# melspectrum007/audio-visual-speech-enhancement

Hardware: NVIDIA B200
Metric: audio-sec/sec (higher is better)
Workload: dtype f32

## Files before the change

audio-visual-speech-enhancement_b200/csrc/avse_common.h:

```cpp
#pragma once

#if defined(__CUDACC__)
#define AVSE_HD __host__ __device__ __forceinline__
#define AVSE_HD_COLD __host__ __device__ __noinline__
#else
#define AVSE_HD inline
#define AVSE_HD_COLD inline
#endif

namespace avse {

constexpr int NFFT = 640;
constexpr int HOP = 160;
constexpr int NBINS = NFFT / 2 + 1;
constexpr int NMEL = 80;
constexpr int SPSS = 20;
constexpr int HALF = NFFT / 2;

constexpr int N1 = 16;
constexpr int N2 = 40;

constexpr int FPG = 2;
constexpr int ROW_F = 84;
constexpr int FRAME_ZERO_F = N1 * ROW_F;
constexpr int FRAME_FLUSH_F = N1 * ROW_F + 16;
constexpr int FRAME_F = FRAME_FLUSH_F + 96;
constexpr int SCAN_BINS = 336;
constexpr int MEL_STAGE_F = 3 * NMEL * FPG;
constexpr int WARP_SMEM_F = FPG * FRAME_F;
static_assert(MEL_STAGE_F <= FRAME_F, "mel staging must fit in one frame buffer");

constexpr int MEL_WMAX = 24;
constexpr int MEL_WROW = 28;
constexpr int MEL_ROUNDS = NMEL / 16;
constexpr int POST_CHUNK = 21;

constexpr float AMIN = 1e-5f;
constexpr float TOP_DB = 80.0f;

#if !defined(AVSE_SPLIT_BLOCKS_FIRST)
#define AVSE_SPLIT_BLOCKS_FIRST 0
#endif
struct WarpSplit {
    long long base;
    int q, r;
    long long extras;
};
inline WarpSplit make_warp_split(long long total, long long blocks, int warps) {
    WarpSplit s;
    const long long nw = blocks * warps;
    s.base = total / nw;
    s.extras = total % nw;
    s.q = (int)(s.extras / blocks);
    s.r = (int)(s.extras % blocks);
    return s;
}
AVSE_HD void warp_split_range(const WarpSplit& s, int block, int warp, int warps, long long& first, long long& count) {
#if AVSE_SPLIT_BLOCKS_FIRST
    const int eb = s.q + (block < s.r ? 1 : 0);
    first = ((long long)block * warps + warp) * s.base + (long long)block * s.q + (block < s.r ? block : s.r) + (warp < eb ? warp : eb);
    count = s.base + (warp < eb ? 1 : 0);
#else
    const long long gw = (long long)block * warps + warp;
    first = gw * s.base + (gw < s.extras ? gw : s.extras);
    count = s.base + (gw < s.extras ? 1 : 0);
#endif
}

#if defined(__CUDACC__)
template <int N4, int THREADS>
struct TableRegs {
    static constexpr int K = (N4 + THREADS - 1) / THREADS;
    float4 v[K];
};
template <int N4, int THREADS>
__device__ __forceinline__ void table_fetch(const void* g, int tid, TableRegs<N4, THREADS>& r) {
#pragma unroll
    for (int k = 0; k < TableRegs<N4, THREADS>::K; ++k) {
        const int i = tid + k * THREADS;
        r.v[k] = i < N4 ? __ldg(reinterpret_cast<const float4*>(g) + i) : make_float4(0.0f, 0.0f, 0.0f, 0.0f);
    }
}
template <int N4, int THREADS>
__device__ __forceinline__ void table_put(float* s, int tid, const TableRegs<N4, THREADS>& r) {
#pragma unroll
    for (int k = 0; k < TableRegs<N4, THREADS>::K; ++k) {
        const int i = tid + k * THREADS;
        if (i < N4) reinterpret_cast<float4*>(s)[i] = r.v[k];
    }
}
template <int N4, int THREADS>
__device__ __forceinline__ void table_put_scaled(float* s, int tid, const TableRegs<N4, THREADS>& r, float scale) {
#pragma unroll
    for (int k = 0; k < TableRegs<N4, THREADS>::K; ++k) {
        const int i = tid + k * THREADS;
        if (i < N4) reinterpret_cast<float4*>(s)[i] = make_float4(r.v[k].x * scale, r.v[k].y * scale, r.v[k].z * scale, r.v[k].w * scale);
    }
}
#endif

}
```

audio-visual-speech-enhancement_b200/csrc/avse_kernels.cu:

```cuda
#include <cuda_runtime.h>
#include <cooperative_groups.h>
#include <cstdio>
#include <cstring>
#include <cstdlib>
#include <string>
#include <vector>
#include <new>

#include "../../include/avse_b200.h"
#include "avse_common.h"
#include "avse_tables.h"
#include "avse_ctx.h"
#include "avse_fwd_stages.cuh"
#include "avse_fwd4_stages.cuh"

using namespace avse;

static thread_local std::string g_err;
int avse_fail(int code, const std::string& msg) { g_err = msg; return code; }
int avse_cuda_fail(cudaError_t e, const char* where) {
    g_err = std::string(where) + ": " + cudaGetErrorString(e);
    return (int)e;
}

// ... 92 lines not shown
    return 0;
}

extern "C" int avse_get_geometry(const avse_ctx* ctx, int* out6) {
    if (ctx == nullptr || out6 == nullptr) return avse_fail(AVSE_E_ARG, "avse_get_geometry: NULL argument");
    out6[0] = ctx->n_fft; out6[1] = ctx->hop; out6[2] = ctx->n_bins; out6[3] = ctx->n_mels; out6[4] = ctx->spss;
    out6[5] = ctx->generic ? 1 : 0;
    return 0;
}

extern "C" int avse_create_ex(int sample_rate, int n_fft, int hop, int n_mels, int spss, double fmin, double fmax, int device,
                              avse_ctx** out) {
    const char* fg = getenv("AVSE_FORCE_GENERIC");
    if (n_fft == NFFT && hop == HOP && n_mels == NMEL && spss == SPSS && !(fg != nullptr && fg[0] == '1')) {
        const int rc = avse_create(sample_rate, fmin, fmax, device, out);
        if (rc != AVSE_E_CONFIG) return rc;
    }
    if (out == nullptr) return avse_fail(AVSE_E_ARG, "avse_create_ex: out is NULL");
    *out = nullptr;
    avse_ctx* c = new (std::nothrow) avse_ctx();
    if (c == nullptr) return avse_fail(AVSE_E_ARG, "avse_create_ex: out of host memory");
    if (!build_generic(c->gen, sample_rate, n_fft, hop, n_mels, spss, fmin, fmax)) {
        std::string e = c->gen.error;
        delete c;
        return avse_fail(AVSE_E_CONFIG, "avse_create_ex: " + e);
    }
    int ndev = 0;
    cudaError_t e = cudaGetDeviceCount(&ndev);
    if (e != cudaSuccess || ndev == 0) { delete c; return avse_fail(AVSE_E_NOCUDA, "avse_create_ex: no CUDA device (this library has no CPU path)"); }
    if (device < 0 || device >= ndev) { delete c; return avse_fail(AVSE_E_ARG, "avse_create_ex: bad device index"); }
    c->device = device;
    c->generic = true;
    c->n_fft = n_fft; c->hop = hop; c->n_bins = c->gen.geo.bins; c->n_mels = n_mels; c->spss = spss;
    int prev = 0;
    cudaGetDevice(&prev);
    CUDA_TRY(cudaSetDevice(device));
    cudaDeviceGetAttribute(&c->num_sms, cudaDevAttrMultiProcessorCount, device);
    const GenericHost& h = c->gen;
    struct Sec { const void* src; size_t bytes; size_t off; };
    std::vector<Sec> secs = {
        {h.window.data(), h.window.size() * 4, 0},         {h.tw.data(), h.tw.size() * 8, 0},
        {h.window_inv.data(), h.window_inv.size() * 4, 0}, {h.tw_inv.data(), h.tw_inv.size() * 8, 0},
        {h.band_lo.data(), h.band_lo.size() * 4, 0},       {h.band_cnt.data(), h.band_cnt.size() * 4, 0},
        {h.band_off.data(), h.band_off.size() * 4, 0},     {h.band_w.data(), h.band_w.size() * 4, 0},
        {h.pinv.data(), h.pinv.size() * 4, 0},
    };
    size_t total = 0;
    for (auto& sc : secs) { sc.off = total; total += (sc.bytes + 255) / 256 * 256; }
    std::vector<char> stage(total, 0);
    for (auto& sc : secs) memcpy(stage.data() + sc.off, sc.src, sc.bytes);
    e = cudaMalloc(&c->gbase, total);
    if (e != cudaSuccess) { delete c; cudaSetDevice(prev); return avse_cuda_fail(e, "cudaMalloc(generic tables)"); }
    e = cudaMemcpy(c->gbase, stage.data(), total, cudaMemcpyHostToDevice);
    if (e != cudaSuccess) { cudaFree(c->gbase); delete c; cudaSetDevice(prev); return avse_cuda_fail(e, "cudaMemcpy(generic tables)"); }
    char* b = (char*)c->gbase;
    c->gd.window = (const float*)(b + secs[0].off);
    c->gd.tw = (const double*)(b + secs[1].off);
    c->gd.window_inv = (const float*)(b + secs[2].off);
    c->gd.tw_inv = (const double*)(b + secs[3].off);
    c->gd.band_lo = (const int*)(b + secs[4].off);
    c->gd.band_cnt = (const int*)(b + secs[5].off);
    c->gd.band_off = (const int*)(b + secs[6].off);
    c->gd.band_w = (const float*)(b + secs[7].off);
    c->gd.pinv = (const float*)(b + secs[8].off);
    cudaSetDevice(prev);
    *out = c;
    return 0;
}

template <typename S> struct Sample4;
template <> struct Sample4<float> {
    typedef float4 vec;
    static __device__ __forceinline__ void load(const float* p, int i, float (&v)[4]) {
        const float4 t = __ldg(reinterpret_cast<const float4*>(p) + i); v[0] = t.x; v[1] = t.y; v[2] = t.z; v[3] = t.w;
    }
};
template <> struct Sample4<short> {
    typedef short4 vec;
    static __device__ __forceinline__ void load(const short* p, int i, float (&v)[4]) {
        const short4 t = __ldg(reinterpret_cast<const short4*>(p) + i); v[0] = t.x; v[1] = t.y; v[2] = t.z; v[3] = t.w;
    }
};

template <typename S, bool CLUSTER>
__global__ void __launch_bounds__(256) avse_snr_factor_kernel(const S* __restrict__ speech, const S* __restrict__ noise,
                                                              long long stride, const int* __restrict__ lengths,
                                                              const int* __restrict__ noise_period, int L,
                                                              const float* __restrict__ snr_db, float* __restrict__ factor_out,
                                                              float* __restrict__ equalizer_out, int* __restrict__ max_key,
                                                              int* __restrict__ min_key) {
    namespace cg = cooperative_groups;
    cg::cluster_group cluster = cg::this_cluster();
    const int P = CLUSTER ? (int)cluster.num_blocks() : 1;
    const int part = CLUSTER ? (int)cluster.block_rank() : 0;
    const int u = blockIdx.x / P;
    int n = lengths ? lengths[u] : L;
    n = n < 0 ? 0 : (n > L ? L : n);
    int Pn = noise_period ? noise_period[u] : n;
    Pn = (Pn <= 0 || Pn > n) ? n : Pn;
    const int q = Pn > 0 ? n / Pn : 0, rem = Pn > 0 ? n - q * Pn : 0;
    const S* s = speech + (size_t)u * stride;
    const S* z = noise + (size_t)u * stride;
    double a0 = 0.0, a1 = 0.0, b0 = 0.0, b1 = 0.0;
    constexpr size_t AL = sizeof(typename Sample4<S>::vec) - 1;
    const int n4 = ((((size_t)s | (size_t)z) & AL) == 0) ? (n >> 2) : 0;
    const int per4 = (n4 + P - 1) / P;
    const int lo4 = part * per4, hi4 = lo4 + per4 < n4 ? lo4 + per4 : n4;
    if (Pn == n) {
        for (int i = lo4 + threadIdx.x; i < hi4; i += blockDim.x) {
            float sv[4], zv[4];
            Sample4<S>::load(s, i, sv);
            Sample4<S>::load(z, i, zv);
            a0 += (double)sv[0] + (double)sv[1] + (double)sv[2] + (double)sv[3];
            a1 += (double)sv[0] * sv[0] + (double)sv[1] * sv[1] + (double)sv[2] * sv[2] + (double)sv[3] * sv[3];
            b0 += (double)zv[0] + (double)zv[1] + (double)zv[2] + (double)zv[3];
            b1 += (double)zv[0] * zv[0] + (double)zv[1] * zv[1] + (double)zv[2] * zv[2] + (double)zv[3] * zv[3];
        }
        if (part == P - 1)
            for (int i = 4 * n4 + threadIdx.x; i < n; i += blockDim.x) {
                const double sv = (double)s[i], zv = (double)z[i];
                a0 += sv; a1 += sv * sv; b0 += zv; b1 += zv * zv;
            }
    } else {
        for (int i = lo4 + threadIdx.x; i < hi4; i += blockDim.x) {
            float sv[4];
            Sample4<S>::load(s, i, sv);
            a0 += (double)sv[0] + (double)sv[1] + (double)sv[2] + (double)sv[3];
            a1 += (double)sv[0] * sv[0] + (double)sv[1] * sv[1] + (double)sv[2] * sv[2] + (double)sv[3] * sv[3];
        }
        if (part == P - 1)
            for (int i = 4 * n4 + threadIdx.x; i < n; i += blockDim.x) { const double sv = (double)s[i]; a0 += sv; a1 += sv * sv; }
        const int perp = (Pn + P - 1) / P;
        const int lop = part * perp, hip = lop + perp < Pn ? lop + perp : Pn;
        for (int i = lop + threadIdx.x; i < hip; i += blockDim.x) {
            const double zv = (double)z[i], w = (double)(q + (i < rem ? 1 : 0));
            b0 += w * zv; b1 += w * zv * zv;
        }
    }
    __shared__ double red[4][8];
    __shared__ double partial[4];
#pragma unroll
    for (int o = 16; o > 0; o >>= 1) {
        a0 += __shfl_xor_sync(0xffffffffu, a0, o);
        a1 += __shfl_xor_sync(0xffffffffu, a1, o);
        b0 += __shfl_xor_sync(0xffffffffu, b0, o);
        b1 += __shfl_xor_sync(0xffffffffu, b1, o);
    }
    const int w = threadIdx.x >> 5, l = threadIdx.x & 31;
    if (l == 0) { red[0][w] = a0; red[1][w] = a1; red[2][w] = b0; red[3][w] = b1; }
    __syncthreads();
    if (threadIdx.x < 4) {
        double t = 0.0;
        for (int i = 0; i < 8; ++i) t += red[threadIdx.x][i];
        partial[threadIdx.x] = t;
    }
    if (CLUSTER) cluster.sync();
    else __syncthreads();
    if (part == 0 && threadIdx.x == 0) {
        double t[4] = {0.0, 0.0, 0.0, 0.0};
        for (int r = 0; r < P; ++r) {
            const double* qq = CLUSTER ? cluster.map_shared_rank(partial, r) : partial;
            t[0] += qq[0]; t[1] += qq[1]; t[2] += qq[2]; t[3] += qq[3];
        }
        float g = 0.0f, f = 0.0f;
        if (n > 0) {
            const double inv = 1.0 / (double)n;
            const double ms = t[0] * inv, mn = t[2] * inv;
            const double vs = t[1] * inv - ms * ms, vn = t[3] * inv - mn * mn;
            const double db = snr_db ? (double)snr_db[u] : 0.0;
            const double eq = sqrt(vs / vn);
            g = (float)eq;
            f = (float)(eq * pow(10.0, -db / 20.0));
        }
        factor_out[u] = f;
        if (equalizer_out) equalizer_out[u] = g;
        if (max_key) { max_key[3 * u] = (int)0x80000000; max_key[3 * u + 1] = (int)0x80000000; max_key[3 * u + 2] = (int)0x80000000; }
        if (min_key) { min_key[3 * u] = 0x7fffffff; min_key[3 * u + 1] = 0x7fffffff; min_key[3 * u + 2] = 0x7fffffff; }
    }
    if (CLUSTER) cluster.sync();
}

template <typename S>
static cudaError_t launch_snr_factor(int B, int P, cudaStream_t st, const S* speech, const S* noise, long long stride, const int* lengths,
                                     const int* noise_period, int L, const float* snr_db, float* factor_out, float* equalizer_out,
                                     int* max_key, int* min_key) {
    if (P == 1) {
        avse_snr_factor_kernel<S, false><<<B, 256, 0, st>>>(speech, noise, stride, lengths, noise_period, L, snr_db, factor_out,
                                                            equalizer_out, max_key, min_key);
        return cudaGetLastError();
    }
    cudaLaunchConfig_t cfg = {};
    cfg.gridDim = dim3((unsigned)(B * P));
    cfg.blockDim = dim3(256);
    cfg.dynamicSmemBytes = 0;
    cfg.stream = st;
    cudaLaunchAttribute attr[1];
    attr[0].id = cudaLaunchAttributeClusterDimension;
    attr[0].val.clusterDim.x = (unsigned)P;
    attr[0].val.clusterDim.y = 1;
    attr[0].val.clusterDim.z = 1;
    cfg.attrs = attr;
    cfg.numAttrs = 1;
    return cudaLaunchKernelEx(&cfg, avse_snr_factor_kernel<S, true>, speech, noise, stride, lengths, noise_period, L, snr_db, factor_out,
                              equalizer_out, max_key, min_key);
}

extern "C" int avse_snr_factor(avse_ctx* ctx, const void* speech, const void* noise, int sample_format, long long stride,
                               const int* lengths, const int* noise_period, int B, int L, const float* snr_db, float* factor_out,
                               float* equalizer_out, int* max_key, int* min_key, void* stream) {
    if (!ctx || !speech || !noise || !factor_out) return avse_fail(AVSE_E_ARG, "avse_snr_factor: NULL argument");
    if (B <= 0 || L <= 0 || stride < L) return avse_fail(AVSE_E_ARG, "avse_snr_factor: bad sizes");
    int P = 1;
    while (P < 8 && (long long)B * P < 4LL * ctx->num_sms && L / (2 * P) >= 65536) P *= 2;
    cudaError_t e;
    if (sample_format == AVSE_SAMPLE_F32)
        e = launch_snr_factor<float>(B, P, (cudaStream_t)stream, (const float*)speech, (const float*)noise, stride, lengths, noise_period, L,
                                     snr_db, factor_out, equalizer_out, max_key, min_key);
    else if (sample_format == AVSE_SAMPLE_I16)
        e = launch_snr_factor<short>(B, P, (cudaStream_t)stream, (const short*)speech, (const short*)noise, stride, lengths, noise_period, L,
                                     snr_db, factor_out, equalizer_out, max_key, min_key);
    else return avse_fail(AVSE_E_ARG, "avse_snr_factor: bad sample_format");
    if (e != cudaSuccess) return avse_cuda_fail(e, "avse_snr_factor launch");
    CUDA_TRY(cudaGetLastError());
    return 0;
}

#ifndef AVSE_FWD_WARPS
#define AVSE_FWD_WARPS 8
#endif
#ifndef AVSE_FWD_CTAS
#define AVSE_FWD_CTAS 2
#endif
constexpr int FWD_WARPS = AVSE_FWD_WARPS;
constexpr int FWD_CTAS = AVSE_FWD_CTAS;
constexpr int FWD_THREADS = FWD_WARPS * 32;
constexpr int FWD_SM_WIN = FWD_WARPS * WARP_SMEM_F;
constexpr int FWD_SM_TW = FWD_SM_WIN + 2 * NFFT;
constexpr int FWD_SM_MODE = FWD_SM_TW + N1 * N2 * 2;
constexpr int FWD_SM_SCANW = FWD_SM_MODE;
constexpr int FWD_SM_SCANMASK = FWD_SM_SCANW + SCAN_BINS * 4;
constexpr int FWD_SM_SCANLOC = FWD_SM_SCANMASK + 16;
constexpr int FWD_SM_MELW = FWD_SM_MODE;
constexpr int FWD_SM_MELLO = FWD_SM_MELW + NMEL * MEL_WROW;
constexpr int FWD_SM_ROUNDW = FWD_SM_MELLO + NMEL;
constexpr int FWD_SMEM_F_SCAN = FWD_SM_SCANLOC + NMEL * 4;
constexpr int FWD_SMEM_F_GEN = FWD_SM_ROUNDW + 16;
constexpr int FWD_SMEM_F = FWD_SMEM_F_GEN > FWD_SMEM_F_SCAN ? FWD_SMEM_F_GEN : FWD_SMEM_F_SCAN;
constexpr int FWD_SMEM_BYTES = FWD_SMEM_F * 4;
static_assert((FWD_SM_MODE % 4) == 0 && (FWD_SM_TW % 2) == 0 && (FWD_SM_SCANLOC % 4) == 0, "table alignment");
static_assert(FWD_CTAS * (FWD_SMEM_BYTES + 1024) <= 233472, "the resident CTAs must fit in shared memory");

struct MixGain { float gain, resid; };
static __device__ __forceinline__ MixGain mix_gain(const avse_forward_args& A, int u) {
    const float f = A.factor ? A.factor[u] : 1.0f;
    MixGain m;
    if (A.equalizer) { m.gain = A.equalizer[u]; m.resid = m.gain != 0.0f ? __fdividef(f, m.gain) : 0.0f; }
    else { m.gain = f; m.resid = 1.0f; }
    return m;
}

struct FwdParams {
    avse_forward_args a;
    FwdTables tb;
    int T;
    int G;
    int total_tiles;
    int per_warp;
    WarpSplit split;
};

template <bool SCAN>
__global__ void __launch_bounds__(FWD_THREADS, FWD_CTAS) avse_forward_kernel(const __grid_constant__ FwdParams P) {
    extern __shared__ __align__(16) float smem[];
    const int warp = threadIdx.x >> 5, lane = threadIdx.x & 31;
    if (SCAN) {
        for (int i = threadIdx.x; i < SCAN_BINS * 4; i += FWD_THREADS) smem[FWD_SM_SCANW + i] = P.tb.scan_w[i];
        if (threadIdx.x < 16) reinterpret_cast<int*>(smem + FWD_SM_SCANMASK)[threadIdx.x] = P.tb.scan_mask[threadIdx.x];
        for (int i = threadIdx.x; i < NMEL * 4; i += FWD_THREADS) reinterpret_cast<int*>(smem + FWD_SM_SCANLOC)[i] = P.tb.scan_loc[i];
    } else {
        for (int i = threadIdx.x; i < NMEL * MEL_WROW; i += FWD_THREADS) smem[FWD_SM_MELW + i] = P.tb.mel_w[i];
        for (int i = threadIdx.x; i < NMEL; i += FWD_THREADS) reinterpret_cast<int*>(smem + FWD_SM_MELLO)[i] = P.tb.mel_lo[i];
        if (threadIdx.x < MEL_ROUNDS) reinterpret_cast<int*>(smem + FWD_SM_ROUNDW)[threadIdx.x] = P.tb.mel_roundw[threadIdx.x];
    }
    for (int i = threadIdx.x; i < 2 * NFFT; i += FWD_THREADS) smem[FWD_SM_WIN + i] = P.tb.window2[i];
    for (int i = threadIdx.x; i < N1 * N2 * 2; i += FWD_THREADS) smem[FWD_SM_TW + i] = P.tb.tw1t[i];
    float* frames = smem + warp * WARP_SMEM_F;
    for (int i = lane; i < WARP_SMEM_F; i += 32) frames[i] = 0.0f;
    __syncthreads();

    const float* s_melw = smem + FWD_SM_MELW;
    const int* s_mello = reinterpret_cast<const int*>(smem + FWD_SM_MELLO);
    const int* s_roundw = reinterpret_cast<const int*>(smem + FWD_SM_ROUNDW);
    const float* s_win = smem + FWD_SM_WIN;
    const vec2* s_tw = reinterpret_cast<const vec2*>(smem + FWD_SM_TW);

    const avse_forward_args& A = P.a;
    const bool have_noise = A.noise != nullptr;
    const int gw = blockIdx.x * FWD_WARPS + warp;
    int tile = gw * P.per_warp;
    int n_tiles = P.total_tiles - tile;
    n_tiles = n_tiles < P.per_warp ? n_tiles : P.per_warp;
    if (n_tiles <= 0) return;
// ... 98 lines not shown
#pragma unroll
                for (int q = 0; q < 3; ++q) stage_db_scan(lane, q, factor, have_noise, s_loc, frames, out, g * FPG, P.T, mx);
            } else {
#pragma unroll
                for (int q = 0; q < 3; ++q) stage_db(lane, q, factor, have_noise, frames, out, g * FPG, P.T, mx);
            }
        }
        __syncwarp();

        if (++g == P.G) {
            flush_max(u);
            g = 0;
            ++u;
            fresh = true;
        }
    }
    if (!fresh) flush_max(u);
}


#ifndef AVSE_P1_UNIFIED
#define AVSE_P1_UNIFIED 0
#endif
#ifndef AVSE_F4_PREFETCH
#define AVSE_F4_PREFETCH 2
#endif
#ifndef AVSE_F4_WARPS
#define AVSE_F4_WARPS 8
#endif
constexpr int F4_WARPS = AVSE_F4_WARPS;
constexpr int F4_THREADS = F4_WARPS * 32;
constexpr int F4_SM_WIN = F4_WARPS * WARP4_SMEM_F;
constexpr int F4_SM_TW = F4_SM_WIN + NFFT;
constexpr int F4_SM_SCANW = F4_SM_TW + N1 * N2 * 2;
constexpr int F4_SM_LOC = F4_SM_SCANW + SCAN4_BINS * 2;
constexpr int F4_SM_MIN = F4_SM_LOC + NMEL * 4;
#ifndef AVSE_F4_PTR_SLOT
#define AVSE_F4_PTR_SLOT 1
#endif
constexpr int F4_UTT_F = AVSE_F4_PTR_SLOT ? 12 : 2;
constexpr int F4_SM_UTT = F4_SM_MIN + F4_WARPS * 96;
constexpr int F4_SMEM_F = F4_SM_UTT + F4_WARPS * 2 * F4_UTT_F;
constexpr int F4_SMEM_BYTES = F4_SMEM_F * 4;
static_assert((F4_SM_TW % 2) == 0 && (F4_SM_SCANW % 2) == 0 && (F4_SM_LOC % 4) == 0 && (F4_SM_UTT % 4) == 0, "table alignment");
static_assert(F4_SMEM_BYTES + 1024 <= 232448, "F4 shared memory must fit in one SM");

#ifndef AVSE_F4_BATCHED_PROLOGUE
#define AVSE_F4_BATCHED_PROLOGUE 1
#endif
__device__ __noinline__ void f4_fill_tables(float* smem, float* frames, const float* window, const float* tw1t, const float* scan4_w,
                                            const int* scan4_loc) {
    static_assert((F4_SM_WIN % 4) == 0 && (F4_SM_TW % 4) == 0 && (F4_SM_SCANW % 4) == 0 && (F4_SM_LOC % 4) == 0 && (WARP4_SMEM_F % 4) == 0, "16-byte table copies");
    const int tid = threadIdx.x, lane = threadIdx.x & 31;
    TableRegs<NFFT / 4, F4_THREADS> r_win;
    TableRegs<N1 * N2 * 2 / 4, F4_THREADS> r_tw;
    TableRegs<SCAN4_BINS * 2 / 4, F4_THREADS> r_sw;
    TableRegs<NMEL, F4_THREADS> r_loc;
    table_fetch(window, tid, r_win);
    table_fetch(tw1t, tid, r_tw);
    table_fetch(scan4_w, tid, r_sw);
    table_fetch(scan4_loc, tid, r_loc);
    for (int i = lane; i < WARP4_SMEM_F / 4; i += 32) reinterpret_cast<float4*>(frames)[i] = make_float4(0.0f, 0.0f, 0.0f, 0.0f);
    table_put(smem + F4_SM_WIN, tid, r_win);
    table_put(smem + F4_SM_TW, tid, r_tw);
    table_put(smem + F4_SM_SCANW, tid, r_sw);
    table_put(smem + F4_SM_LOC, tid, r_loc);
}

template <typename S, bool TILED, bool PAD>
__global__ void __launch_bounds__(F4_THREADS, 1) avse_forward4_kernel(const __grid_constant__ FwdParams P) {
    extern __shared__ __align__(16) float smem[];
    const int warp = threadIdx.x >> 5, lane = threadIdx.x & 31;
    float* frames = smem + warp * WARP4_SMEM_F;
#if AVSE_F4_BATCHED_PROLOGUE
    f4_fill_tables(smem, frames, P.tb.window, P.tb.tw1t, P.tb.scan4_w, P.tb.scan4_loc);
#else
    for (int i = threadIdx.x; i < NFFT; i += F4_THREADS) smem[F4_SM_WIN + i] = P.tb.window[i];
    for (int i = threadIdx.x; i < N1 * N2 * 2; i += F4_THREADS) smem[F4_SM_TW + i] = P.tb.tw1t[i];
    for (int i = threadIdx.x; i < SCAN4_BINS * 2; i += F4_THREADS) smem[F4_SM_SCANW + i] = P.tb.scan4_w[i];
    for (int i = threadIdx.x; i < NMEL * 4; i += F4_THREADS) reinterpret_cast<int*>(smem + F4_SM_LOC)[i] = P.tb.scan4_loc[i];
    for (int i = lane; i < WARP4_SMEM_F; i += 32) frames[i] = 0.0f;
#endif
    __syncthreads();

    const float* s_win = smem + F4_SM_WIN;
    const vec2* s_tw = reinterpret_cast<const vec2*>(smem + F4_SM_TW);
    const vec2* s_scanw = reinterpret_cast<const vec2*>(smem + F4_SM_SCANW);
    const ivec4* s_loc = reinterpret_cast<const ivec4*>(smem + F4_SM_LOC);

    Lane4Const lc;
    lane4_const_init(lane, s_win, s_tw, lc);
    const unsigned mask_lo = P.tb.scan4_mask[2 * (lane & 7)], mask_hi = P.tb.scan4_mask[2 * (lane & 7) + 1];

    const avse_forward_args& A = P.a;
    long long first, count;
    warp_split_range(P.split, (int)blockIdx.x, warp, F4_WARPS, first, count);
    int tile = (int)first;
    const int n_tiles = (int)count;
    if (n_tiles <= 0) return;
    int u = tile / P.G;
    int g = tile - u * P.G;

    float mx[3] = {neg_inf(), neg_inf(), neg_inf()};
    float* mn = smem + F4_SM_MIN + warp * 96;
    mn[lane] = -neg_inf(); mn[32 + lane] = -neg_inf(); mn[64 + lane] = -neg_inf();
    float factor = 0.0f;
    int vs = 0, vn = 0;
    float* utt_sm = smem + F4_SM_UTT + warp * (2 * F4_UTT_F);
    const S* in_speech = reinterpret_cast<const S*>(A.speech);
    const S* in_noise = reinterpret_cast<const S*>(A.noise);
    constexpr int LINE = 128 / (int)sizeof(S);

    auto flush_max = [&](int uu) {
#pragma unroll
        for (int s = 0; s < 3; ++s) {
            float v = mx[s], w = mn[32 * s + lane];
#pragma unroll
            for (int o = 16; o > 0; o >>= 1) {
                v = fmaxf(v, __shfl_xor_sync(0xffffffffu, v, o));
                w = fminf(w, __shfl_xor_sync(0xffffffffu, w, o));
            }
            if (lane == 0) {
                atomicMax(A.max_key + 3 * uu + s, float_to_key(v));
                if (A.min_key) atomicMin(A.min_key + 3 * uu + s, float_to_key(w));
            }
            mx[s] = neg_inf();
            mn[32 * s + lane] = -neg_inf();
        }
    };

    auto prefetch_ahead = [&](int it, int u, int g) {
#if AVSE_F4_PREFETCH > 0
        if (it + AVSE_F4_PREFETCH < n_tiles) {
            int g2 = g + AVSE_F4_PREFETCH, u2 = u;
            if (g2 >= P.G) { g2 -= P.G; ++u2; }
            const int lo = g2 == 0 ? 0 : g2 * (F4 * HOP) + HOP;
            const int hi = g2 * (F4 * HOP) + (NFFT + HOP);
            const int i0 = (lo & ~(LINE - 1)) + LINE * lane;
            if (i0 < hi && i0 < A.L && i0 < A.in_stride && lane < 22) {
                const size_t o = (size_t)u2 * A.in_stride + i0;
                asm volatile("prefetch.global.L2 [%0];" ::"l"(in_speech + o));
                asm volatile("prefetch.global.L2 [%0];" ::"l"(in_noise + o));
            }
        }
#endif
    };
    auto load_utt = [&](int uu, int& ovs, int& ovn, float& of) {
        ovs = A.len_speech ? A.len_speech[uu] : A.L;
        ovn = A.len_noise ? A.len_noise[uu] : ovs;
        ovs = ovs < 0 ? 0 : (ovs < A.L ? ovs : A.L);
        ovn = ovn < 0 ? 0 : (ovn < A.L ? ovn : A.L);
        const MixGain mg = mix_gain(A, uu);
        of = mg.resid;
        utt_sm[F4_UTT_F * (uu & 1)] = mg.gain;
#if AVSE_F4_PTR_SLOT
        {
            float** ps = reinterpret_cast<float**>(utt_sm + F4_UTT_F * (uu & 1) + 2);
            ps[0] = A.out_speech ? A.out_speech + (size_t)uu * A.out_stride : nullptr;
            ps[1] = A.out_noise ? A.out_noise + (size_t)uu * A.out_stride : nullptr;
            ps[2] = A.out_mixed ? A.out_mixed + (size_t)uu * A.out_stride : nullptr;
            ps[3] = A.mixed_pcm ? A.mixed_pcm + (size_t)uu * A.pcm_stride : nullptr;
        }
#endif
        if (TILED) {
            int period = A.noise_period[uu];
            if (period <= 0 || period >= ovn) period = 0;
// ... 93 lines not shown
            out.dst[1] = A.out_noise ? A.out_noise + (size_t)u * A.out_stride : nullptr;
            out.dst[2] = A.out_mixed ? A.out_mixed + (size_t)u * A.out_stride : nullptr;
#endif
            out.layout = A.layout;
            out.n_slices = A.n_slices;
            out.ld_t = A.ld_t;
#pragma unroll 1
#if AVSE_DB_SPLIT_LAST && AVSE_DB_BRANCHFREE_EXTRA
            for (int q = 0; q < 2; ++q) stage4_db(lane, q, tl.factor, s_loc, frames, out, g * F4, P.T, mx, mn);
            stage4_db_last(lane, tl.factor, s_loc, frames, out, g * F4, P.T, mx, mn);
#else
            for (int q = 0; q < 3; ++q) stage4_db(lane, q, tl.factor, s_loc, frames, out, g * F4, P.T, mx, mn);
#endif
        }
        __syncwarp();

        if (last_of_utt || !have_next) flush_max(u);
        u = u2; g = g2; vs = vs2; vn = vn2;
        tl = tnx;
        interior = interior2;
        reflect = reflect2;
    }
}

__global__ void avse_reset_max_kernel(int* __restrict__ max_key, int* __restrict__ min_key, int n, int min_value);

extern "C" int avse_forward(avse_ctx* ctx, const avse_forward_args* args, void* stream) {
    if (!ctx || !args) return avse_fail(AVSE_E_ARG, "avse_forward: NULL argument");
    if (ctx->generic) return avse_generic_forward(ctx, args, stream);
    const avse_forward_args& a = *args;
    if (!a.speech || !a.max_key) return avse_fail(AVSE_E_ARG, "avse_forward: speech and max_key are required");
    if (a.B <= 0 || a.L <= HALF) return avse_fail(AVSE_E_ARG, "avse_forward: need B > 0 and L > 320 (reflect padding)");
    if (!a.len_speech && a.in_stride < a.L) return avse_fail(AVSE_E_ARG, "avse_forward: in_stride < L needs len_speech");
    if (a.layout != AVSE_LAYOUT_SLICES && a.layout != AVSE_LAYOUT_SPEC) return avse_fail(AVSE_E_ARG, "avse_forward: bad layout");
    FwdParams P;
    P.a = a;
    P.tb = ctx->fwd;
    P.T = 1 + a.L / HOP;
    P.G = (P.T + FPG - 1) / FPG;
    if (a.layout == AVSE_LAYOUT_SLICES) {
        if (a.n_slices < 0 || (long long)a.n_slices * AVSE_SPSS > P.T) return avse_fail(AVSE_E_ARG, "avse_forward: n_slices exceeds int(T/20) (dp:50)");
        if (a.out_stride < (long long)a.n_slices * NMEL * AVSE_SPSS) return avse_fail(AVSE_E_ARG, "avse_forward: out_stride too small");
    } else {
        if (a.ld_t < P.T) return avse_fail(AVSE_E_ARG, "avse_forward: ld_t < T");
        if (a.out_stride < (long long)NMEL * a.ld_t) return avse_fail(AVSE_E_ARG, "avse_forward: out_stride too small");
    }
    if (a.mixed_pcm && a.pcm_stride < a.L) return avse_fail(AVSE_E_ARG, "avse_forward: pcm_stride < L");
    float* outs[3] = {a.out_speech, a.out_noise, a.out_mixed};
    for (int s = 0; s < 3; ++s)
        if (outs[s] && (((size_t)outs[s] & 15) || (a.out_stride & 3))) return avse_fail(AVSE_E_ARG, "avse_forward: outputs must be 16-byte aligned with out_stride % 4 == 0");
    const long long total = (long long)a.B * P.G;
    if (total > 0x7fffffffLL) return avse_fail(AVSE_E_ARG, "avse_forward: B * groups exceeds 2^31; split the batch");

    static thread_local int configured_dev = -1;
    int dev = 0;
    CUDA_TRY(cudaGetDevice(&dev));
    if (dev != ctx->device) return avse_fail(AVSE_E_ARG, "avse_forward: current device differs from the context's device");
    if (a.sample_format != AVSE_SAMPLE_F32 && a.sample_format != AVSE_SAMPLE_I16) return avse_fail(AVSE_E_ARG, "avse_forward: bad sample_format");
    const bool i16 = a.sample_format == AVSE_SAMPLE_I16;
    const bool use_f4 = ctx->f4_tables && a.noise != nullptr && a.stft_speech == nullptr && (!ctx->force_f2 || i16);
    if (i16 && !use_f4) return avse_fail(AVSE_E_ARG, "avse_forward: int16 samples are supported for pair batches (noise != NULL, no stft_speech) with the standard 2-tap filterbank; convert to float32 first");
    if (use_f4) {
        static thread_local int configured4_dev = -1;
        if (configured4_dev != dev) {
            CUDA_TRY(cudaFuncSetAttribute(avse_forward4_kernel<float, false, false>, cudaFuncAttributeMaxDynamicSharedMemorySize, F4_SMEM_BYTES));
            CUDA_TRY(cudaFuncSetAttribute(avse_forward4_kernel<short, false, false>, cudaFuncAttributeMaxDynamicSharedMemorySize, F4_SMEM_BYTES));
            CUDA_TRY(cudaFuncSetAttribute(avse_forward4_kernel<float, false, true>, cudaFuncAttributeMaxDynamicSharedMemorySize, F4_SMEM_BYTES));
            CUDA_TRY(cudaFuncSetAttribute(avse_forward4_kernel<short, false, true>, cudaFuncAttributeMaxDynamicSharedMemorySize, F4_SMEM_BYTES));
            CUDA_TRY(cudaFuncSetAttribute(avse_forward4_kernel<float, true, false>, cudaFuncAttributeMaxDynamicSharedMemorySize, F4_SMEM_BYTES));
            CUDA_TRY(cudaFuncSetAttribute(avse_forward4_kernel<short, true, false>, cudaFuncAttributeMaxDynamicSharedMemorySize, F4_SMEM_BYTES));
            configured4_dev = dev;
        }
        P.G = (P.T + F4 - 1) / F4;
        const long long total4 = (long long)a.B * P.G;
        long long blocks4 = ctx->num_sms;
        const long long need4 = (total4 + F4_WARPS - 1) / F4_WARPS;
        if (blocks4 > need4) blocks4 = need4;
        const long long nwarps4 = blocks4 * F4_WARPS;
        P.total_tiles = (int)total4;
        P.per_warp = (int)((total4 + nwarps4 - 1) / nwarps4);
        P.split = make_warp_split(total4, blocks4, F4_WARPS);
        const bool tiled = a.noise_period != nullptr;
        const bool pad = !tiled && (a.len_speech != nullptr || a.len_noise != nullptr);
        const cudaStream_t st4 = (cudaStream_t)stream;
        if (i16 && tiled) avse_forward4_kernel<short, true, false><<<(unsigned)blocks4, F4_THREADS, F4_SMEM_BYTES, st4>>>(P);
        else if (tiled) avse_forward4_kernel<float, true, false><<<(unsigned)blocks4, F4_THREADS, F4_SMEM_BYTES, st4>>>(P);
        else if (i16 && pad) avse_forward4_kernel<short, false, true><<<(unsigned)blocks4, F4_THREADS, F4_SMEM_BYTES, st4>>>(P);
        else if (pad) avse_forward4_kernel<float, false, true><<<(unsigned)blocks4, F4_THREADS, F4_SMEM_BYTES, st4>>>(P);
        else if (i16) avse_forward4_kernel<short, false, false><<<(unsigned)blocks4, F4_THREADS, F4_SMEM_BYTES, st4>>>(P);
        else avse_forward4_kernel<float, false, false><<<(unsigned)blocks4, F4_THREADS, F4_SMEM_BYTES, st4>>>(P);
        CUDA_TRY(cudaGetLastError());
        return 0;
    }
    if (configured_dev != dev) {
        CUDA_TRY(cudaFuncSetAttribute(avse_forward_kernel<true>, cudaFuncAttributeMaxDynamicSharedMemorySize, FWD_SMEM_BYTES));
        CUDA_TRY(cudaFuncSetAttribute(avse_forward_kernel<false>, cudaFuncAttributeMaxDynamicSharedMemorySize, FWD_SMEM_BYTES));
        configured_dev = dev;
    }
    long long blocks = (long long)FWD_CTAS * ctx->num_sms;
    const long long need = (total + FWD_WARPS - 1) / FWD_WARPS;
    if (blocks > need) blocks = need;
    const long long nwarps = blocks * FWD_WARPS;
    P.total_tiles = (int)total;
    P.per_warp = (int)((total + nwarps - 1) / nwarps);
    if (ctx->std_tables) avse_forward_kernel<true><<<(unsigned)blocks, FWD_THREADS, FWD_SMEM_BYTES, (cudaStream_t)stream>>>(P);
    else avse_forward_kernel<false><<<(unsigned)blocks, FWD_THREADS, FWD_SMEM_BYTES, (cudaStream_t)stream>>>(P);
    CUDA_TRY(cudaGetLastError());
    if (a.min_key) {
        avse_reset_max_kernel<<<(3 * a.B + 255) / 256, 256, 0, (cudaStream_t)stream>>>(nullptr, a.min_key, 3 * a.B, (int)0x80000000);
        CUDA_TRY(cudaGetLastError());
    }
    return 0;
}

#ifndef AVSE_FLOOR_ZLOOP
#define AVSE_FLOOR_ZLOOP 1
#endif
static __device__ __forceinline__ void floor_store(float4* q, float4 v, float thr) {
    if (fminf(fminf(v.x, v.y), fminf(v.z, v.w)) < thr) {
        v.x = fmaxf(v.x, thr); v.y = fmaxf(v.y, thr); v.z = fmaxf(v.z, thr); v.w = fmaxf(v.w, thr);
        *q = v;
    }
}

__global__ void __launch_bounds__(256) avse_floor_inplace_kernel(float* __restrict__ data0, float* __restrict__ data1,
                                                                 float* __restrict__ data2, long long stride, long long n_per_utt,
                                                                 const int* __restrict__ max_key, const int* __restrict__ min_key,
                                                                 int which0, int n_sig) {
    const int u = blockIdx.x;
#if AVSE_FLOOR_ZLOOP
    for (int z = 0; z < n_sig; ++z) {
#else
    const int z = blockIdx.z;
    {
#endif
    float* data = z == 0 ? data0 : (z == 1 ? data1 : data2);
    const float thr = key_to_float(max_key[3 * u + which0 + z]) - TOP_DB;
#if AVSE_FLOOR_ZLOOP
    if (min_key != nullptr && key_to_float(min_key[3 * u + which0 + z]) >= thr) continue;
#else
    if (min_key != nullptr && key_to_float(min_key[3 * u + which0 + z]) >= thr) return;
#endif
    float* p = data + (size_t)u * stride;
    const long long n4 = n_per_utt >> 2;
    const long long step = (long long)gridDim.y * blockDim.x;
    long long i = (long long)blockIdx.y * blockDim.x + threadIdx.x;
    for (; i + 3 * step < n4; i += 4 * step) {
        float4* q = reinterpret_cast<float4*>(p) + i;
        const float4 v0 = q[0], v1 = q[step], v2 = q[2 * step], v3 = q[3 * step];
        floor_store(q, v0, thr);
        floor_store(q + step, v1, thr);
        floor_store(q + 2 * step, v2, thr);
        floor_store(q + 3 * step, v3, thr);
    }
    for (; i < n4; i += step) {
        float4 v = reinterpret_cast<float4*>(p)[i];
        if (fminf(fminf(v.x, v.y), fminf(v.z, v.w)) < thr) {
            v.x = fmaxf(v.x, thr); v.y = fmaxf(v.y, thr); v.z = fmaxf(v.z, thr); v.w = fmaxf(v.w, thr);
            reinterpret_cast<float4*>(p)[i] = v;
        }
    }
    for (long long j = 4 * n4 + (long long)blockIdx.y * blockDim.x + threadIdx.x; j < n_per_utt; j += step)
        p[j] = fmaxf(p[j], thr);
    }
}

static unsigned floor_grid_x(long long n_per_utt) {
    long long bx = (n_per_utt / 4 + 256 * 8 - 1) / (256 * 8);
    if (bx < 1) bx = 1;
    if (bx > 256) bx = 256;
    return (unsigned)bx;
}

extern "C" int avse_floor_inplace3(avse_ctx* ctx, float* speech, float* noise, float* mixed, long long stride, long long n_per_utt,
                                   int B, const int* max_key, const int* min_key, void* stream) {
    if (!ctx || !speech || !noise || !mixed || !max_key) return avse_fail(AVSE_E_ARG, "avse_floor_inplace3: NULL argument");
    if (B <= 0 || n_per_utt <= 0 || stride < n_per_utt) return avse_fail(AVSE_E_ARG, "avse_floor_inplace3: bad sizes");
    if ((((size_t)speech | (size_t)noise | (size_t)mixed) & 15) || (stride & 3))
        return avse_fail(AVSE_E_ARG, "avse_floor_inplace3: data must be 16-byte aligned with stride % 4 == 0");
    dim3 grid((unsigned)B, floor_grid_x(n_per_utt), AVSE_FLOOR_ZLOOP ? 1 : 3);
    avse_floor_inplace_kernel<<<grid, 256, 0, (cudaStream_t)stream>>>(speech, noise, mixed, stride, n_per_utt, max_key, min_key, 0, 3);
    CUDA_TRY(cudaGetLastError());
    return 0;
}

extern "C" int avse_floor_inplace(avse_ctx* ctx, float* data, long long stride, long long n_per_utt, int B, const int* max_key,
                                  const int* min_key, int which, void* stream) {
    if (!ctx || !data || !max_key) return avse_fail(AVSE_E_ARG, "avse_floor_inplace: NULL argument");
    if (B <= 0 || n_per_utt <= 0 || stride < n_per_utt || which < 0 || which > 2) return avse_fail(AVSE_E_ARG, "avse_floor_inplace: bad sizes");
    if (((size_t)data & 15) || (stride & 3)) return avse_fail(AVSE_E_ARG, "avse_floor_inplace: data must be 16-byte aligned with stride % 4 == 0");
    dim3 grid((unsigned)B, floor_grid_x(n_per_utt));
    avse_floor_inplace_kernel<<<grid, 256, 0, (cudaStream_t)stream>>>(data, data, data, stride, n_per_utt, max_key, min_key, which, 1);
    CUDA_TRY(cudaGetLastError());
    return 0;
}

__global__ void __launch_bounds__(256) avse_floor_gather_kernel(const float* __restrict__ spec, long long spec_stride, int ld_t,
                                                                float* __restrict__ slices, long long slices_stride, int n_slices,
                                                                const int* __restrict__ max_key, int which, int n_mels, int spss) {
    const int u = blockIdx.x;
    const float thr = key_to_float(max_key[3 * u + which]) - TOP_DB;
    const float* src = spec + (size_t)u * spec_stride;
    float* dst = slices + (size_t)u * slices_stride;
    const int n = n_slices * n_mels * spss;
    for (int i = blockIdx.y * blockDim.x + threadIdx.x; i < n; i += gridDim.y * blockDim.x) {
        const int j = i % spss;
        const int m = (i / spss) % n_mels;
        const int s = i / (spss * n_mels);
        dst[i] = fmaxf(src[(size_t)m * ld_t + s * spss + j], thr);
    }
}

extern "C" int avse_floor_gather(avse_ctx* ctx, const float* spec, long long spec_stride, int ld_t, float* slices,
                                 long long slices_stride, int n_slices, int B, const int* max_key, int which, void* stream) {
    if (!ctx || !spec || !slices || !max_key) return avse_fail(AVSE_E_ARG, "avse_floor_gather: NULL argument");
    if (B <= 0 || n_slices <= 0 || ld_t < n_slices * ctx->spss || which < 0 || which > 2) return avse_fail(AVSE_E_ARG, "avse_floor_gather: bad sizes");
    const int n = n_slices * ctx->n_mels * ctx->spss;
    int bx = (n + 255) / 256;
    if (bx > 64) bx = 64;
    dim3 grid((unsigned)B, (unsigned)bx);
    avse_floor_gather_kernel<<<grid, 256, 0, (cudaStream_t)stream>>>(spec, spec_stride, ld_t, slices, slices_stride, n_slices, max_key, which,
                                                                     ctx->n_mels, ctx->spss);
    CUDA_TRY(cudaGetLastError());
    return 0;
}

__global__ void avse_reset_max_kernel(int* __restrict__ max_key, int* __restrict__ min_key, int n, int min_value) {
    const int i = blockIdx.x * blockDim.x + threadIdx.x;
    if (i < n) {
        if (max_key) max_key[i] = (int)0x80000000;
        if (min_key) min_key[i] = min_value;
    }
}

extern "C" int avse_reset_max(avse_ctx* ctx, int* max_key, int* min_key, int n, void* stream) {
    if (!ctx || !max_key || n <= 0) return avse_fail(AVSE_E_ARG, "avse_reset_max: bad argument");
    avse_reset_max_kernel<<<(n + 255) / 256, 256, 0, (cudaStream_t)stream>>>(max_key, min_key, n, 0x7fffffff);
    CUDA_TRY(cudaGetLastError());
    return 0;
}

__global__ void avse_max_db_kernel(const int* __restrict__ max_key, int n, float* __restrict__ out) {
    const int i = blockIdx.x * blockDim.x + threadIdx.x;
    if (i < n) out[i] = key_to_float(max_key[i]);
}

extern "C" int avse_max_db(avse_ctx* ctx, const int* max_key, int n, float* out_db, void* stream) {
    if (!ctx || !max_key || !out_db || n <= 0) return avse_fail(AVSE_E_ARG, "avse_max_db: bad argument");
    avse_max_db_kernel<<<(n + 255) / 256, 256, 0, (cudaStream_t)stream>>>(max_key, n, out_db);
    CUDA_TRY(cudaGetLastError());
    return 0;
}

__global__ void __launch_bounds__(256) avse_gather_rows_kernel(const float* __restrict__ s0, const float* __restrict__ s1,
                                                               const float* __restrict__ s2, long long src_rows,
                                                               const long long* __restrict__ index, long long n_out, int row4,
                                                               float* __restrict__ d0, float* __restrict__ d1, float* __restrict__ d2,
                                                               int* __restrict__ bad) {
    const int z = blockIdx.y;
    const float4* src = reinterpret_cast<const float4*>(z == 0 ? s0 : (z == 1 ? s1 : s2));
    float4* dst = reinterpret_cast<float4*>(z == 0 ? d0 : (z == 1 ? d1 : d2));
    const int lane = threadIdx.x & 31;
    const long long warp = ((long long)blockIdx.x * blockDim.x + threadIdx.x) >> 5;
    const long long nwarps = ((long long)gridDim.x * blockDim.x) >> 5;
    for (long long i = warp; i < n_out; i += nwarps) {
        const long long r = index[i];
        if (r < 0 || r >= src_rows) { if (lane == 0) atomicExch(bad, 1); continue; }
        const float4* sp = src + r * row4;
        float4* dp = dst + i * row4;
        int j = lane;
        for (; j + 96 < row4; j += 128) {
            const float4 a = sp[j], b = sp[j + 32], c = sp[j + 64], d = sp[j + 96];
            dp[j] = a; dp[j + 32] = b; dp[j + 64] = c; dp[j + 96] = d;
        }
        for (; j < row4; j += 32) dp[j] = sp[j];
    }
// ... 25 lines not shown
```

Before: 4.732 million.

## Enable programmatic dependent launch across kernels and retune floor and SNR grids

Adds griddepcontrol wait and launch_dependents calls and launches the SNR, forward and floor kernels with programmatic stream serialization, so each kernel's prologue can overlap the tail of the one before it. The floor kernel grid is now sized from the SM count and batch size rather than a fixed cap, its loop uses pointer arithmetic, and minimum-CTA launch bounds are added to it and to the small-batch SNR kernel. The aim is to cut launch gaps and tail effects between short kernels. The risk is an incorrect PDL ordering, and the higher occupancy hints could limit registers.

Result: faster. 4.807 million, median of 6 (+1.6%).

```diff
diff --git a/audio-visual-speech-enhancement_b200/csrc/avse_common.h b/audio-visual-speech-enhancement_b200/csrc/avse_common.h
--- a/audio-visual-speech-enhancement_b200/csrc/avse_common.h
+++ b/audio-visual-speech-enhancement_b200/csrc/avse_common.h
@@ -68,6 +68,34 @@
 }
 
 #if defined(__CUDACC__)
+#if !defined(AVSE_PDL)
+#define AVSE_PDL 1
+#endif
+__device__ __forceinline__ void pdl_wait() {
+#if AVSE_PDL
+    asm volatile("griddepcontrol.wait;" ::: "memory");
+#endif
+}
+__device__ __forceinline__ void pdl_launch_dependents() {
+#if AVSE_PDL
+    asm volatile("griddepcontrol.launch_dependents;");
+#endif
+}
+template <typename... KArgs, typename... Args>
+inline cudaError_t launch_pdl(void (*kernel)(KArgs...), dim3 grid, dim3 block, size_t smem, cudaStream_t st, Args&&... args) {
+    cudaLaunchConfig_t cfg = {};
+    cfg.gridDim = grid;
+    cfg.blockDim = block;
+    cfg.dynamicSmemBytes = smem;
+    cfg.stream = st;
+    cudaLaunchAttribute attr[1];
+    attr[0].id = cudaLaunchAttributeProgrammaticStreamSerialization;
+    attr[0].val.programmaticStreamSerializationAllowed = 1;
+    cfg.attrs = attr;
+    cfg.numAttrs = AVSE_PDL ? 1 : 0;
+    return cudaLaunchKernelEx(&cfg, kernel, static_cast<Args&&>(args)...);
+}
+
 template <int N4, int THREADS>
 struct TableRegs {
     static constexpr int K = (N4 + THREADS - 1) / THREADS;
diff --git a/audio-visual-speech-enhancement_b200/csrc/avse_kernels.cu b/audio-visual-speech-enhancement_b200/csrc/avse_kernels.cu
--- a/audio-visual-speech-enhancement_b200/csrc/avse_kernels.cu
+++ b/audio-visual-speech-enhancement_b200/csrc/avse_kernels.cu
@@ -198,8 +198,8 @@
     }
 };
 
-template <typename S, bool CLUSTER>
-__global__ void __launch_bounds__(256) avse_snr_factor_kernel(const S* __restrict__ speech, const S* __restrict__ noise,
+template <typename S, bool CLUSTER, int MIN_CTAS>
+__global__ void __launch_bounds__(256, MIN_CTAS) avse_snr_factor_kernel(const S* __restrict__ speech, const S* __restrict__ noise,
                                                               long long stride, const int* __restrict__ lengths,
                                                               const int* __restrict__ noise_period, int L,
                                                               const float* __restrict__ snr_db, float* __restrict__ factor_out,
@@ -210,6 +210,7 @@
     const int P = CLUSTER ? (int)cluster.num_blocks() : 1;
     const int part = CLUSTER ? (int)cluster.block_rank() : 0;
     const int u = blockIdx.x / P;
+    pdl_wait();
     int n = lengths ? lengths[u] : L;
     n = n < 0 ? 0 : (n > L ? L : n);
     int Pn = noise_period ? noise_period[u] : n;
@@ -253,6 +254,7 @@
             b0 += w * zv; b1 += w * zv * zv;
         }
     }
+    pdl_launch_dependents();
     __shared__ double red[4][8];
     __shared__ double partial[4];
 #pragma unroll
@@ -297,13 +299,12 @@
 }
 
 template <typename S>
-static cudaError_t launch_snr_factor(int B, int P, cudaStream_t st, const S* speech, const S* noise, long long stride, const int* lengths,
-                                     const int* noise_period, int L, const float* snr_db, float* factor_out, float* equalizer_out,
-                                     int* max_key, int* min_key) {
+static cudaError_t launch_snr_factor(int B, int P, int num_sms, cudaStream_t st, const S* speech, const S* noise, long long stride,
+                                     const int* lengths, const int* noise_period, int L, const float* snr_db, float* factor_out,
+                                     float* equalizer_out, int* max_key, int* min_key) {
     if (P == 1) {
-        avse_snr_factor_kernel<S, false><<<B, 256, 0, st>>>(speech, noise, stride, lengths, noise_period, L, snr_db, factor_out,
-                                                            equalizer_out, max_key, min_key);
-        return cudaGetLastError();
+        return launch_pdl(B <= 8 * num_sms ? avse_snr_factor_kernel<S, false, 8> : avse_snr_factor_kernel<S, false, 0>, dim3(B), dim3(256), 0, st,
+                          speech, noise, stride, lengths, noise_period, L, snr_db, factor_out, equalizer_out, max_key, min_key);
     }
     cudaLaunchConfig_t cfg = {};
     cfg.gridDim = dim3((unsigned)(B * P));
@@ -317,7 +318,7 @@
     attr[0].val.clusterDim.z = 1;
     cfg.attrs = attr;
     cfg.numAttrs = 1;
-    return cudaLaunchKernelEx(&cfg, avse_snr_factor_kernel<S, true>, speech, noise, stride, lengths, noise_period, L, snr_db, factor_out,
+    return cudaLaunchKernelEx(&cfg, avse_snr_factor_kernel<S, true, 0>, speech, noise, stride, lengths, noise_period, L, snr_db, factor_out,
                               equalizer_out, max_key, min_key);
 }
 
@@ -330,10 +331,10 @@
     while (P < 8 && (long long)B * P < 4LL * ctx->num_sms && L / (2 * P) >= 65536) P *= 2;
     cudaError_t e;
     if (sample_format == AVSE_SAMPLE_F32)
-        e = launch_snr_factor<float>(B, P, (cudaStream_t)stream, (const float*)speech, (const float*)noise, stride, lengths, noise_period, L,
+        e = launch_snr_factor<float>(B, P, ctx->num_sms, (cudaStream_t)stream, (const float*)speech, (const float*)noise, stride, lengths, noise_period, L,
                                      snr_db, factor_out, equalizer_out, max_key, min_key);
     else if (sample_format == AVSE_SAMPLE_I16)
-        e = launch_snr_factor<short>(B, P, (cudaStream_t)stream, (const short*)speech, (const short*)noise, stride, lengths, noise_period, L,
+        e = launch_snr_factor<short>(B, P, ctx->num_sms, (cudaStream_t)stream, (const short*)speech, (const short*)noise, stride, lengths, noise_period, L,
                                      snr_db, factor_out, equalizer_out, max_key, min_key);
     else return avse_fail(AVSE_E_ARG, "avse_snr_factor: bad sample_format");
     if (e != cudaSuccess) return avse_cuda_fail(e, "avse_snr_factor launch");
@@ -598,6 +599,7 @@
     for (int i = lane; i < WARP4_SMEM_F; i += 32) frames[i] = 0.0f;
 #endif
     __syncthreads();
+    pdl_wait();
 
     const float* s_win = smem + F4_SM_WIN;
     const vec2* s_tw = reinterpret_cast<const vec2*>(smem + F4_SM_TW);
@@ -857,14 +859,11 @@
         P.split = make_warp_split(total4, blocks4, F4_WARPS);
         const bool tiled = a.noise_period != nullptr;
         const bool pad = !tiled && (a.len_speech != nullptr || a.len_noise != nullptr);
-        const cudaStream_t st4 = (cudaStream_t)stream;
-        if (i16 && tiled) avse_forward4_kernel<short, true, false><<<(unsigned)blocks4, F4_THREADS, F4_SMEM_BYTES, st4>>>(P);
-        else if (tiled) avse_forward4_kernel<float, true, false><<<(unsigned)blocks4, F4_THREADS, F4_SMEM_BYTES, st4>>>(P);
-        else if (i16 && pad) avse_forward4_kernel<short, false, true><<<(unsigned)blocks4, F4_THREADS, F4_SMEM_BYTES, st4>>>(P);
-        else if (pad) avse_forward4_kernel<float, false, true><<<(unsigned)blocks4, F4_THREADS, F4_SMEM_BYTES, st4>>>(P);
-        else if (i16) avse_forward4_kernel<short, false, false><<<(unsigned)blocks4, F4_THREADS, F4_SMEM_BYTES, st4>>>(P);
-        else avse_forward4_kernel<float, false, false><<<(unsigned)blocks4, F4_THREADS, F4_SMEM_BYTES, st4>>>(P);
-        CUDA_TRY(cudaGetLastError());
+        void (*kern)(const FwdParams) = i16 ? (tiled ? avse_forward4_kernel<short, true, false>
+                                                     : (pad ? avse_forward4_kernel<short, false, true> : avse_forward4_kernel<short, false, false>))
+                                           : (tiled ? avse_forward4_kernel<float, true, false>
+                                                     : (pad ? avse_forward4_kernel<float, false, true> : avse_forward4_kernel<float, false, false>));
+        CUDA_TRY(launch_pdl(kern, dim3((unsigned)blocks4), dim3(F4_THREADS), F4_SMEM_BYTES, (cudaStream_t)stream, P));
         return 0;
     }
     if (configured_dev != dev) {
@@ -898,11 +897,13 @@
     }
 }
 
-__global__ void __launch_bounds__(256) avse_floor_inplace_kernel(float* __restrict__ data0, float* __restrict__ data1,
+__global__ void __launch_bounds__(256, 8) avse_floor_inplace_kernel(float* __restrict__ data0, float* __restrict__ data1,
                                                                  float* __restrict__ data2, long long stride, long long n_per_utt,
                                                                  const int* __restrict__ max_key, const int* __restrict__ min_key,
                                                                  int which0, int n_sig) {
     const int u = blockIdx.x;
+    pdl_wait();
+    pdl_launch_dependents();
 #if AVSE_FLOOR_ZLOOP
     for (int z = 0; z < n_sig; ++z) {
 #else
@@ -917,33 +918,28 @@
     if (min_key != nullptr && key_to_float(min_key[3 * u + which0 + z]) >= thr) return;
 #endif
     float* p = data + (size_t)u * stride;
-    const long long n4 = n_per_utt >> 2;
-    const long long step = (long long)gridDim.y * blockDim.x;
-    long long i = (long long)blockIdx.y * blockDim.x + threadIdx.x;
-    for (; i + 3 * step < n4; i += 4 * step) {
-        float4* q = reinterpret_cast<float4*>(p) + i;
+    const int step = (int)(gridDim.y * blockDim.x);
+    const int t = (int)(blockIdx.y * blockDim.x + threadIdx.x);
+    float4* const end = reinterpret_cast<float4*>(p) + (n_per_utt >> 2);
+    float4* q = reinterpret_cast<float4*>(p) + t;
+    for (; end - q > 3LL * step; q += 4 * step) {
         const float4 v0 = q[0], v1 = q[step], v2 = q[2 * step], v3 = q[3 * step];
         floor_store(q, v0, thr);
         floor_store(q + step, v1, thr);
         floor_store(q + 2 * step, v2, thr);
         floor_store(q + 3 * step, v3, thr);
     }
-    for (; i < n4; i += step) {
-        float4 v = reinterpret_cast<float4*>(p)[i];
-        if (fminf(fminf(v.x, v.y), fminf(v.z, v.w)) < thr) {
-            v.x = fmaxf(v.x, thr); v.y = fmaxf(v.y, thr); v.z = fmaxf(v.z, thr); v.w = fmaxf(v.w, thr);
-            reinterpret_cast<float4*>(p)[i] = v;
-        }
-    }
-    for (long long j = 4 * n4 + (long long)blockIdx.y * blockDim.x + threadIdx.x; j < n_per_utt; j += step)
+    for (; q < end; q += step) floor_store(q, *q, thr);
+    for (long long j = 4 * (n_per_utt >> 2) + t; j < n_per_utt; j += step)
         p[j] = fmaxf(p[j], thr);
     }
 }
 
-static unsigned floor_grid_x(long long n_per_utt) {
-    long long bx = (n_per_utt / 4 + 256 * 8 - 1) / (256 * 8);
+static unsigned floor_grid_x(long long n_per_utt, int B, int num_sms) {
+    long long bx = 8LL * num_sms / B;
+    const long long most = (n_per_utt / 4 + 256 * 4 - 1) / (256 * 4);
+    if (bx > most) bx = most;
     if (bx < 1) bx = 1;
-    if (bx > 256) bx = 256;
     return (unsigned)bx;
 }
 
@@ -953,9 +949,9 @@
     if (B <= 0 || n_per_utt <= 0 || stride < n_per_utt) return avse_fail(AVSE_E_ARG, "avse_floor_inplace3: bad sizes");
     if ((((size_t)speech | (size_t)noise | (size_t)mixed) & 15) || (stride & 3))
         return avse_fail(AVSE_E_ARG, "avse_floor_inplace3: data must be 16-byte aligned with stride % 4 == 0");
-    dim3 grid((unsigned)B, floor_grid_x(n_per_utt), AVSE_FLOOR_ZLOOP ? 1 : 3);
-    avse_floor_inplace_kernel<<<grid, 256, 0, (cudaStream_t)stream>>>(speech, noise, mixed, stride, n_per_utt, max_key, min_key, 0, 3);
-    CUDA_TRY(cudaGetLastError());
+    const dim3 grid((unsigned)B, floor_grid_x(n_per_utt, B, ctx->num_sms), AVSE_FLOOR_ZLOOP ? 1 : 3);
+    CUDA_TRY(launch_pdl(avse_floor_inplace_kernel, grid, dim3(256), 0, (cudaStream_t)stream, speech, noise, mixed, stride, n_per_utt, max_key,
+                        min_key, 0, 3));
     return 0;
 }
 
@@ -964,9 +960,9 @@
     if (!ctx || !data || !max_key) return avse_fail(AVSE_E_ARG, "avse_floor_inplace: NULL argument");
     if (B <= 0 || n_per_utt <= 0 || stride < n_per_utt || which < 0 || which > 2) return avse_fail(AVSE_E_ARG, "avse_floor_inplace: bad sizes");
     if (((size_t)data & 15) || (stride & 3)) return avse_fail(AVSE_E_ARG, "avse_floor_inplace: data must be 16-byte aligned with stride % 4 == 0");
-    dim3 grid((unsigned)B, floor_grid_x(n_per_utt));
-    avse_floor_inplace_kernel<<<grid, 256, 0, (cudaStream_t)stream>>>(data, data, data, stride, n_per_utt, max_key, min_key, which, 1);
-    CUDA_TRY(cudaGetLastError());
+    const dim3 grid((unsigned)B, floor_grid_x(n_per_utt, B, ctx->num_sms));
+    CUDA_TRY(launch_pdl(avse_floor_inplace_kernel, grid, dim3(256), 0, (cudaStream_t)stream, data, data, data, stride, n_per_utt, max_key,
+                        min_key, which, 1));
     return 0;
 }
 
```
